# Dizzy-cell/HOUV

Measured on AMD Instinct MI355X. Metric: registration pairs/sec (2048-pt partial pairs), higher is better.
Workload: dtype f32; 1 GPU; HOUV solve_model, 2048x2048-pt pairs, batch 256/GPU, K=64 restarts x 200 Adam iterations + retry stages (BASELINE configs[1]); pairs_per_gpu=256, points=2048, kernel=64, iters=200, icp_refine=False, parallelism=dp1 (pair shards, one RCCL all-gather of [steps*P,12] per rank)

## Files before the change

### houv_amd/csrc/capi.hip

```cpp
#include <stdarg.h>
#include <string.h>

#include "../../include/houv_hip.h"
#include "houv_common.h"

namespace houv {

static thread_local char g_err[512] = "";

void set_error(const char* fmt, ...) {
  va_list ap;
  va_start(ap, fmt);
  vsnprintf(g_err, sizeof(g_err), fmt, ap);
  va_end(ap);
  fprintf(stderr, "[houv_hip] %s\n", g_err);
}

DebugKnobs g_debug;

namespace {

__global__ void pose_kernel(const float* __restrict__ params, int n, int angle_base, int trans_mode,
                            float* __restrict__ R, float* __restrict__ T) {
  const int i = blockIdx.x * blockDim.x + threadIdx.x;
  if (i >= n) return;
  float p[8];
#pragma unroll
  for (int k = 0; k < 8; ++k) p[k] = params[i * 8 + k];
  Pose f;
  pose_forward(p, angle_base, trans_mode, f);
#pragma unroll
  for (int k = 0; k < 9; ++k) R[i * 9 + k] = f.R[k];
#pragma unroll
  for (int k = 0; k < 3; ++k) T[i * 3 + k] = f.T[k];
}

__global__ void move_kernel(const float* __restrict__ src, const float* __restrict__ R, const float* __restrict__ T,
                            size_t total, int N, float* __restrict__ moved) {
  for (size_t e = (size_t)blockIdx.x * blockDim.x + threadIdx.x; e < total; e += (size_t)gridDim.x * blockDim.x) {
    const size_t b = e / N;
    const float* r = R + b * 9;
    const float x = src[e * 3 + 0], y = src[e * 3 + 1], z = src[e * 3 + 2];
    moved[e * 3 + 0] = __builtin_fmaf(z, r[2], __builtin_fmaf(y, r[1], x * r[0])) + T[b * 3 + 0];
    moved[e * 3 + 1] = __builtin_fmaf(z, r[5], __builtin_fmaf(y, r[4], x * r[3])) + T[b * 3 + 1];
    moved[e * 3 + 2] = __builtin_fmaf(z, r[8], __builtin_fmaf(y, r[7], x * r[6])) + T[b * 3 + 2];
  }
}

}
}

extern "C" int houv_abi_version(void) { return HOUV_ABI_VERSION; }

extern "C" const char* houv_last_error(void) { return houv::g_err; }

extern "C" int houv_debug_set(const char* name, long long value) {
  using namespace houv;
  const struct { const char* name; std::atomic<int>* knob; long long lo, hi, step; } ints[] = {
      {"solve_predict", &g_debug.pred_mode, 0, 2, 1}, {"knn_split", &g_debug.knn_split, 0, 1, 1},
      {"attn_split", &g_debug.attn_split, 0, 1, 1},   {"gemm_split", &g_debug.gemm_split, 0, 6, 3}};
  if (name && !strcmp(name, "solve_stats")) {
    g_debug.stats = (unsigned long long)value;
    return 1;
  }
  if (name && !strcmp(name, "solve_walk_hist")) {
    g_debug.walk_hist = (unsigned long long)value;
    return 1;
  }
  if (name && !strcmp(name, "solve_cull_stats")) {
    g_debug.cull_stats = (unsigned long long)value;
    return 1;
  }
  for (const auto& k : ints)
    if (name && !strcmp(name, k.name) && value >= k.lo && value <= k.hi && value % k.step == 0) {
      *k.knob = (int)value;
      return 1;
    }
  set_error("houv_debug_set: unknown switch or value out of range: %s = %lld", name ? name : "(null)", value);
  return 0;
}

#ifndef HOUV_BUILD_ID
#define HOUV_BUILD_ID "unknown"
#endif
extern "C" const char* houv_build_id(void) { return HOUV_BUILD_ID; }

extern "C" int houv_pose_forward(const float* params, int n, int angle_base, int trans_mode, const float* src, int N,
                                 float* R, float* T, float* moved, void* stream) {
  using namespace houv;
  if (n < 0 || !params || !R || !T || angle_base < 0 || angle_base > 3 || trans_mode < 0 || trans_mode > 1) {
    set_error("houv_pose_forward: bad argument");
    return 0;
  }
  if (n == 0) return 1;
  hipStream_t s = (hipStream_t)stream;
  pose_kernel<<<(n + 255) / 256, 256, 0, s>>>(params, n, angle_base, trans_mode, R, T);
  if (src && moved && N > 0) {
    const size_t total = (size_t)n * N;
    size_t blocks = (total + 255) / 256;
    if (blocks > 16384) blocks = 16384;
    move_kernel<<<(unsigned)blocks, 256, 0, s>>>(src, R, T, total, N, moved);
  }
  return check_launch("houv_pose_forward") ? 1 : 0;
}
```

### houv_amd/csrc/houv_common.h

```cpp
#pragma once
#include <hip/hip_runtime.h>
#include <stdint.h>
#include <stdio.h>

#include <atomic>

#include "houv_math.h"

namespace houv {

constexpr int kWave = 64;
constexpr int kSub = 32;
constexpr int kTrk = 16;

void set_error(const char* fmt, ...);
struct SolveCommon;
__attribute__((visibility("hidden"))) int solve_check_args(const char* who, const SolveCommon& a, int use_views);
__attribute__((visibility("hidden"))) bool scatter_index_launch(const int* keys, int B, int N, int M, int* offsets, int* order,
                                                                hipStream_t stream);
inline bool check_launch(const char* what) {
  hipError_t e = hipGetLastError();
  if (e != hipSuccess) {
    set_error("%s: %s", what, hipGetErrorString(e));
    return false;
  }
  return true;
}

struct DebugKnobs {
  std::atomic<int> pred_mode{0};
  std::atomic<unsigned long long> stats{0ull};
  std::atomic<unsigned long long> walk_hist{0ull};
  std::atomic<unsigned long long> cull_stats{0ull};
  std::atomic<int> knn_split{1};
  std::atomic<int> attn_split{1};
  std::atomic<int> gemm_split{6};
};
extern DebugKnobs g_debug;

template <int MET>
__device__ __forceinline__ float metric_sqdist(float dx, float dy, float dz) {
  if constexpr (MET == 0) return __builtin_fmaf(dz, dz, __builtin_fmaf(dy, dy, dx * dx));
  else if constexpr (MET == 1) return __builtin_fmaf(dz, dz, dy * dy);
  else if constexpr (MET == 2) return __builtin_fmaf(dz, dz, dx * dx);
  else return __builtin_fmaf(dy, dy, dx * dx);
}

__device__ __forceinline__ float min3f(float a, float b, float c) {
  return __builtin_fminf(__builtin_fminf(a, b), c);
}

__device__ __forceinline__ float wave_sum(float v) {
#pragma unroll
  for (int o = 32; o > 0; o >>= 1) v += __shfl_xor(v, o, kWave);
  return v;
}

__device__ __forceinline__ int wave_sum_i(int v) {
#pragma unroll
  for (int o = 32; o > 0; o >>= 1) v += __shfl_xor(v, o, kWave);
  return v;
}

template <int CTRL, int ROW_MASK = 0xf, int BANK_MASK = 0xf>
__device__ __forceinline__ float dpp_f(float v) {
  return __int_as_float(__builtin_amdgcn_update_dpp(0, __float_as_int(v), CTRL, ROW_MASK, BANK_MASK, true));
}
template <int CTRL, int ROW_MASK = 0xf, int BANK_MASK = 0xf>
__device__ __forceinline__ int dpp_i(int v) {
  return __builtin_amdgcn_update_dpp(0, v, CTRL, ROW_MASK, BANK_MASK, true);
}

__device__ __forceinline__ float wave_sum_to_lane63(float v) {
  v += dpp_f<0x111>(v);
  v += dpp_f<0x112>(v);
  v += dpp_f<0x114>(v);
  v += dpp_f<0x118>(v);
  v += dpp_f<0x142, 0xa>(v);
  v += dpp_f<0x143, 0xc>(v);
  return v;
}

__device__ __forceinline__ int wave_max_to_lane63(int v) {
  v = max(v, dpp_i<0x111>(v));
  v = max(v, dpp_i<0x112>(v));
  v = max(v, dpp_i<0x114>(v));
  v = max(v, dpp_i<0x118>(v));
  v = max(v, dpp_i<0x142, 0xa>(v));
  v = max(v, dpp_i<0x143, 0xc>(v));
  return v;
}

template <int CTRL, int ROW_MASK = 0xf>
__device__ __forceinline__ float fmax_dpp(float v) {
  return __builtin_fmaxf(v, __int_as_float(__builtin_amdgcn_update_dpp(__float_as_int(v), __float_as_int(v), CTRL, ROW_MASK, 0xf, false)));
}
__device__ __forceinline__ float wave_fmax_to_lane63(float v) {
  v = fmax_dpp<0x111>(v);
  v = fmax_dpp<0x112>(v);
  v = fmax_dpp<0x114>(v);
  v = fmax_dpp<0x118>(v);
  v = fmax_dpp<0x142, 0xa>(v);
  v = fmax_dpp<0x143, 0xc>(v);
  return v;
}

__device__ __forceinline__ int wave_incl_scan_dpp(int x) {
  int v = x + dpp_i<0x111>(x);
  v += dpp_i<0x112>(x);
  v += dpp_i<0x113>(x);
  v += dpp_i<0x114, 0xf, 0xe>(v);
  v += dpp_i<0x118, 0xf, 0xc>(v);
  v += dpp_i<0x142, 0xa>(v);
  v += dpp_i<0x143, 0xc>(v);
  return v;
}

__device__ __forceinline__ int wave_incl_scan_i(int v) {
  const int lane = threadIdx.x & 63;
#pragma unroll
  for (int o = 1; o < 64; o <<= 1) {
    int n = __shfl_up(v, o, kWave);
    if (lane >= o) v += n;
  }
  return v;
}

}
```

### houv_amd/csrc/houv_solve.h

```cpp
#pragma once
#include <stddef.h>

#include "houv_sweep.h"

namespace houv {

struct SolveCommon {
  const float* src;
  const float* tgt;
  int P, N, M, K;
  double* state;
  int steps_done, n_iters, angle_base, trans_mode, f64_params, k_full, k_view;
  double lr, beta1, beta2, eps;
  float loss_scale;
  float* out_score;
  float* out_loss;
  float* out_R;
  float* out_T;
  float* out_grad;
  float* out_cd;
};

constexpr int kRedStride = 4 * kAccN;
constexpr int kHistBins = 256;
constexpr int kHistSets = 3;
constexpr int kPoseFloats = 28;
static_assert(sizeof(Pose) <= kPoseFloats * 4 && offsetof(Pose, T) == 36, "pose[0..11] in LDS must be R | T");

__device__ __forceinline__ void store_pose(float* dst, const Pose& f) {
  const float* src = reinterpret_cast<const float*>(&f);
#pragma unroll
  for (int i = 0; i < (int)(sizeof(Pose) / 4); ++i) dst[i] = src[i];
}
__device__ __forceinline__ void load_pose(Pose& f, const float* src) {
  float* dst = reinterpret_cast<float*>(&f);
#pragma unroll
  for (int i = 0; i < (int)(sizeof(Pose) / 4); ++i) dst[i] = src[i];
}
__device__ __forceinline__ void load_rt(const float* pose, float (&R)[9], float (&T)[3]) {
#pragma unroll
  for (int i = 0; i < 9; ++i) R[i] = pose[i];
#pragma unroll
  for (int i = 0; i < 3; ++i) T[i] = pose[9 + i];
}

__device__ __forceinline__ void move_point(const float (&R)[9], const float (&T)[3], float sx, float sy, float sz, float& mx,
                                           float& my, float& mz) {
  mx = __builtin_fmaf(sz, R[2], __builtin_fmaf(sy, R[1], sx * R[0])) + T[0];
  my = __builtin_fmaf(sz, R[5], __builtin_fmaf(sy, R[4], sx * R[3])) + T[1];
  mz = __builtin_fmaf(sz, R[8], __builtin_fmaf(sy, R[7], sx * R[6])) + T[2];
}

__device__ __forceinline__ void store_outputs(float* out_score, float* out_loss, float* out_R, float* out_T, float* out_grad,
                                              float* out_cd, int inst, const Pose& f, const TailLoss& r) {
  if (out_score) out_score[inst] = r.score;
  if (out_loss) out_loss[inst] = r.loss;
  if (out_R)
    for (int k = 0; k < 9; ++k) out_R[(size_t)inst * 9 + k] = f.R[k];
  if (out_T)
    for (int k = 0; k < 3; ++k) out_T[(size_t)inst * 3 + k] = f.T[k];
  if (out_grad)
    for (int k = 0; k < 8; ++k) out_grad[(size_t)inst * 8 + k] = r.g[k];
  if (out_cd)
    for (int m = 0; m < 4; ++m)
      for (int d = 0; d < 2; ++d) out_cd[(size_t)inst * 8 + m * 2 + d] = r.cd[m][d];
}

struct RadixState {
  unsigned prefix, mask;
  int remaining, neq;
};

template <int BLOCK>
__device__ __forceinline__ unsigned* radix_rotate(unsigned* hist, int& hrot, int tid) {
  unsigned* h = hist + hrot * kHistBins;
  hrot = (hrot == kHistSets - 1) ? 0 : hrot + 1;
  for (int i = tid; i < kHistBins; i += BLOCK) hist[hrot * kHistBins + i] = 0u;
  return h;
}

__device__ __forceinline__ void radix_count(unsigned* h, unsigned key, int pass, int lane, const RadixState& s) {
  if (pass == 0) {
    const unsigned digit = key >> 24;
    unsigned long long todo = __ballot(1);
    while (todo) {
      const int leader = __ffsll((long long)todo) - 1;
      const unsigned d = (unsigned)__builtin_amdgcn_readlane((int)digit, leader);
      const unsigned long long m = __ballot(digit == d);
      if (lane == leader) atomicAdd(&h[d], (unsigned)__popcll(m));
      todo &= ~m;
    }
  } else if ((key & s.mask) == s.prefix) {
    atomicAdd(&h[(key >> (24 - 8 * pass)) & 255u], 1u);
  }
}

__device__ __forceinline__ void radix_pick(const unsigned* h, int pass, int lane, RadixState& s) {
  const int shift = 24 - 8 * pass;
  const uint4 hv = *reinterpret_cast<const uint4*>(h + 4 * lane);
  const int hh[4] = {(int)hv.x, (int)hv.y, (int)hv.z, (int)hv.w};
  const int tot = hh[0] + hh[1] + hh[2] + hh[3];
  int c = wave_incl_scan_dpp(tot) - tot;
  int fbin = 0, fc = 0, fn = 0;
  bool found = false;
#pragma unroll
  for (int b = 0; b < 4; ++b) {
    const bool hit = c < s.remaining && s.remaining <= c + hh[b];
    fbin = hit ? 4 * lane + b : fbin;
    fc = hit ? c : fc;
    fn = hit ? hh[b] : fn;
    found = found || hit;
    c += hh[b];
  }
  const int src_lane = __ffsll((long long)__ballot(found)) - 1;
  const int bin = __builtin_amdgcn_readlane(fbin, src_lane);
  s.prefix |= (unsigned)bin << shift;
  s.mask |= 255u << shift;
  s.remaining -= __builtin_amdgcn_readlane(fc, src_lane);
  s.neq = __builtin_amdgcn_readlane(fn, src_lane);
}

}
```

### houv_amd/csrc/solve.hip

```cpp
#include <stddef.h>
#include <stdlib.h>

#include "../../include/houv_hip.h"
#include "houv_common.h"
#include "houv_solve.h"

namespace houv {
namespace {

struct SolveArgs : SolveCommon {
  short* nn_ws;
  int ws_valid;
  int ws_stride;
  int pred_mode;
  unsigned long long* stats;
  unsigned long long* walk_hist;
  unsigned long long* cull_stats;
};

constexpr int kRescanBatch = 4;
constexpr int kRefresh = 4;
constexpr int kTermMaxAge = 0;

struct Smem {
  float4* tgt;
  float4* mov;
  double* state;
  double* adam;
  float* pose;
  float* acc;
  float* red;
  unsigned* hist;
  int* ctl;
  float4* tbox;
  float4* mbox;
  SortedStage st;
  float* anchor;
};
constexpr int kAnchorFloats = kTermAnchorFloats + 4;
constexpr int kTermAges = 8;
constexpr int kStalePose = 4;


__host__ __device__ inline int pad_unit(int prune) { return prune == 3 ? 2 * kSub : kSub; }

__host__ __device__ inline size_t smem_bytes(int N, int M, int block, int prune, int q) {
  const int pu = pad_unit(prune);
  int npad = (N + pu - 1) / pu * pu, mpad = (M + pu - 1) / pu * pu;
  if (prune) npad = mpad = (npad > mpad ? npad : mpad);
  const int nw = block / 64;
  const size_t nq = (size_t)block * q;
  return (size_t)(npad + mpad) * 16 + 28 * 8 + kPoseFloats * 4 + 8 * kAccStride * 4 + (size_t)2 * nw * kRedStride * 4 +
         kHistSets * kHistBins * 4 + (8 + nw) * 4 + 64 + (prune ? 2 * 128 * 16 + nq * 2 + 132 * 4 + kAnchorFloats * 4 : 0);
}

__device__ inline Smem carve(unsigned char* base, int N, int M, int block, int nq, int pu) {
  int npad = (N + pu - 1) / pu * pu, mpad = (M + pu - 1) / pu * pu;
  if (nq) npad = mpad = (npad > mpad ? npad : mpad);
  const int nw = block / 64;
  Smem s;
  s.tgt = reinterpret_cast<float4*>(base);
  s.mov = s.tgt + mpad;
  s.state = reinterpret_cast<double*>(s.mov + npad);
  s.adam = s.state + 24;
  s.pose = reinterpret_cast<float*>(s.adam + 4);
  s.acc = s.pose + kPoseFloats;
  s.red = s.acc + 8 * kAccStride;
  s.hist = reinterpret_cast<unsigned*>(s.red + 2 * nw * kRedStride);
  s.ctl = reinterpret_cast<int*>(s.hist + kHistSets * kHistBins);
  const size_t box_off = ((size_t)(reinterpret_cast<unsigned char*>(s.ctl + 8 + nw) - base) + 15) & ~(size_t)15;
  s.tbox = reinterpret_cast<float4*>(base + box_off);
  s.mbox = s.tbox + 128;
  s.st.hist = reinterpret_cast<int*>(s.mbox + 128);
  s.st.order = reinterpret_cast<unsigned short*>(s.st.hist + 132);
  s.anchor = reinterpret_cast<float*>(s.st.order + nq);
  return s;
}

template <typename T>
__device__ __forceinline__ T fresh(T v) {
  asm volatile("" : "+s"(v));
  return v;
}
__device__ __forceinline__ const float* fresh_lds(const float* p) {
  typedef const float __attribute__((address_space(3))) * lds_f;
  return (const float*)(lds_f)(size_t)fresh((unsigned)(size_t)(lds_f)p);
}

template <int BLOCK, int Q>
__device__ __forceinline__ void select_smallest(const unsigned (&key)[Q], int ksel, unsigned* hist, int* ctl,
                                                bool (&sel)[Q], int& hrot) {
  constexpr int NW = BLOCK / 64;
  const int tid = tid_x(), lane = tid & 63, wave = tid >> 6;
  RadixState rs{0u, 0u, ksel, 0};
#pragma unroll
  for (int pass = 0; pass < 4; ++pass) {
    unsigned* h = radix_rotate<BLOCK>(hist, hrot, tid);
#pragma unroll
    for (int k = 0; k < Q; ++k) radix_count(h, key[k], pass, lane, rs);
    __syncthreads();
    radix_pick(h, pass, lane, rs);
  }
  const unsigned prefix = rs.prefix;
  const int remaining = rs.remaining, neq = rs.neq;
  if (neq == remaining) {
#pragma unroll
    for (int k = 0; k < Q; ++k) sel[k] = key[k] <= prefix;
  } else {
    int e = 0;
#pragma unroll
    for (int k = 0; k < Q; ++k) e += (key[k] == prefix) ? 1 : 0;
    const int incl = wave_incl_scan_dpp(e);
    __syncthreads();
    if (lane == 63) ctl[8 + wave] = incl;
    __syncthreads();
    int rank = incl - e;
    for (int w = 0; w < NW; ++w) rank += (w < wave) ? ctl[8 + w] : 0;
#pragma unroll
    for (int k = 0; k < Q; ++k) {
      const bool eq = key[k] == prefix;
      sel[k] = key[k] < prefix || (eq && rank < remaining);
      rank += eq ? 1 : 0;
    }
  }
}

constexpr int kGradN = 12;

__device__ __forceinline__ void park(float v, float* dst) {
  v = wave_sum_to_lane63(v);
  if ((tid_x() & 63) == 63) *dst = v;
}

template <int BLOCK, int Q, int NMET>
__device__ __forceinline__ void select_all(const Smem& sm, const float (&best)[Q][NMET], int count, int k_full, int k_view,
                                           unsigned need, int& hrot, unsigned (&bits)[NMET]) {
  bool valid[Q], sel[Q];
  unsigned key[Q];
#pragma unroll
  for (int m = 0; m < NMET; ++m) {
    const int ksel = (m == 0) ? k_full : k_view;
#pragma unroll
    for (int k = 0; k < Q; ++k) {
      valid[k] = pt_index<BLOCK>(k) < count;
      key[k] = valid[k] ? __float_as_uint(best[k][m]) : 0xFFFFFFFFu;
      sel[k] = valid[k];
    }
    if (ksel < count && ((need >> m) & 1u)) select_smallest<BLOCK, Q>(key, ksel, sm.hist, sm.ctl, sel, hrot);
    unsigned b = 0u;
#pragma unroll
    for (int k = 0; k < Q; ++k) b |= sel[k] ? (1u << k) : 0u;
    bits[m] = b;
  }
}

template <int Q>
__device__ __forceinline__ float lane_sqrt_sum(const float (&bd)[Q], unsigned selbits) {
  float s = 0.f;
#pragma unroll
  for (int k = 0; k < Q; ++k)
    if ((selbits >> k) & 1u) s += (bd[k] < INFINITY) ? sqrtf(bd[k]) : NAN;
  return s;
}

template <int BLOCK, int Q, int MET, int DIR, bool WS>
__device__ __forceinline__ void lane_grad_sums(const Smem& sm, const float4* __restrict__ refs, const float (&qx)[Q],
                                               const float (&qy)[Q], const float (&qz)[Q], const float (&bd)[Q],
                                               const int (&bt)[Q], unsigned selbits, int count, const float (&px)[Q],
                                               const float (&py)[Q], const float (&pz)[Q], float (&g)[kGradN], buf_t ws,
                                               int ws_off) {
  const int rot = tid_x() & (kSub - 1);
#pragma unroll
  for (int i = 0; i < kGradN; ++i) g[i] = 0.f;
  float R[9], T[3];
  if constexpr (DIR == 0) load_rt(sm.pose, R, T);
#pragma unroll
  for (int k = 0; k < Q; ++k) {
    int jn;
    const float4 nn = recover_nn<MET, kRescanBatch, true>(refs + bt[k] * kTrk, qx[k], qy[k], qz[k], bd[k], rot, jn);
    if (WS && pt_index<BLOCK>(k) < count)
      __builtin_amdgcn_raw_buffer_store_b16((unsigned short)(bt[k] * kTrk + jn), ws, tid_x() * kNnRec,
                                            ws_off + pt_base<BLOCK>(k) * kNnRec + MET * 2, 0);
    if ((selbits >> k) & 1u) {
      const float s = (bd[k] < INFINITY) ? sqrtf(bd[k]) : NAN;
      const float inv = 1.0f / s;
      float dx, dy, dz, sx, sy, sz;
      if constexpr (DIR == 1) {
        dx = qx[k] - nn.x; dy = qy[k] - nn.y; dz = qz[k] - nn.z;
        sx = px[k]; sy = py[k]; sz = pz[k];
      } else {
        dx = nn.x - qx[k]; dy = nn.y - qy[k]; dz = nn.z - qz[k];
        const float ux = nn.x - T[0], uy = nn.y - T[1], uz = nn.z - T[2];
        sx = R[0] * ux + R[3] * uy + R[6] * uz;
        sy = R[1] * ux + R[4] * uy + R[7] * uz;
        sz = R[2] * ux + R[5] * uy + R[8] * uz;
      }
      if constexpr (MET == 1) dx = 0.f;
      if constexpr (MET == 2) dy = 0.f;
      if constexpr (MET == 3) dz = 0.f;
      const float cx = dx * inv, cy = dy * inv, cz = dz * inv;
      g[0] += cx; g[1] += cy; g[2] += cz;
      g[3] += cx * sx; g[4] += cx * sy; g[5] += cx * sz;
      g[6] += cy * sx; g[7] += cy * sy; g[8] += cy * sz;
      g[9] += cz * sx; g[10] += cz * sy; g[11] += cz * sz;
    }
  }
}

template <int BLOCK, int Q, int NMET>
__device__ __forceinline__ void park_sqrt_sums(const float (&best)[Q][NMET], const unsigned (&selbits)[NMET], unsigned need,
                                               float* red_wave) {
  float bd[Q];
#pragma unroll
  for (int m = 0; m < NMET; ++m) {
    if (!((need >> m) & 1u)) continue;
#pragma unroll
    for (int k = 0; k < Q; ++k) bd[k] = best[k][m];
    park(lane_sqrt_sum<Q>(bd, selbits[m]), red_wave + m * kAccN);
  }
}

template <int BLOCK, int Q, int NMET, int DIR, bool WS>
__device__ __forceinline__ void park_grad_sums(const Smem& sm, const float4* __restrict__ refs, const float (&qx)[Q],
                                               const float (&qy)[Q], const float (&qz)[Q], const float (&best)[Q][NMET],
                                               const int (&btile)[Q][NMET], const unsigned (&selbits)[NMET], unsigned mask,
                                               int count, const float (&px)[Q], const float (&py)[Q], const float (&pz)[Q],
                                               float* red_wave, buf_t ws, int ws_off) {
  float bd[Q], g[kGradN];
  int bt[Q];
#define HOUV_GRAD(MET)                                                                                              \
  if ((mask >> MET) & 1u) {                                                                                         \
    _Pragma("unroll") for (int k = 0; k < Q; ++k) {                                                                 \
      bd[k] = best[k][MET];                                                                                         \
      bt[k] = btile[k][MET];                                                                                        \
    }                                                                                                               \
    lane_grad_sums<BLOCK, Q, MET, DIR, WS>(sm, refs, qx, qy, qz, bd, bt, selbits[MET], count, px, py, pz, g,        \
                                           ws, ws_off);                                                             \
    _Pragma("unroll") for (int i = 0; i < kGradN; ++i) park(g[i], red_wave + MET * kAccN + 1 + i);                  \
  }
  HOUV_GRAD(0)
  if constexpr (NMET == 4) {
    HOUV_GRAD(1)
    HOUV_GRAD(2)
    HOUV_GRAD(3)
  }
#undef HOUV_GRAD
}

template <int BLOCK, int NMET>
__device__ __forceinline__ void final_sums(const Smem& sm, int dir, bool want_s, unsigned grad_mask, unsigned need) {
  constexpr int NW = BLOCK / 64;
  const int tid = tid_x();
  if (tid < NMET * kAccN) {
    const int m = tid / kAccN, i = tid % kAccN;
    if ((i == 0) ? want_s : (((grad_mask >> m) & 1u) != 0u)) {
      const float* r = sm.red + (size_t)dir * NW * kRedStride + tid;
      float a = 0.f;
#pragma unroll
      for (int w = 0; w < NW; ++w) a += r[w * kRedStride];
      if (i == 0 && !((need >> m) & 1u)) a = INFINITY;
      sm.acc[(m * 2 + dir) * kAccStride + i] = a;
    }
  }
}

template <int NMET>
__device__ __forceinline__ unsigned picked_direction(const Smem& sm, int k_full, int k_view) {
  unsigned pick = 0u;
#pragma unroll
  for (int m = 0; m < NMET; ++m) {
    const float kk = (float)((m == 0) ? k_full : k_view);
    const float cd0 = sm.acc[(m * 2 + 0) * kAccStride] / kk, cd1 = sm.acc[(m * 2 + 1) * kAccStride] / kk;
    pick |= (cd0 <= cd1) ? 0u : (1u << m);
  }
  return pick;
}

template <int BLOCK>
__device__ __forceinline__ void load_src_point(buf_t src, int k, int N, float& x, float& y, float& z) {
  x = y = z = 0.f;
  if (pt_index<BLOCK>(k) < N) {
    const auto v = __builtin_amdgcn_raw_buffer_load_b96(src, tid_x() * 12, pt_base<BLOCK>(k) * 12, 0);
    x = __uint_as_float(v[0]); y = __uint_as_float(v[1]); z = __uint_as_float(v[2]);
  }
}

template <int BLOCK, int Q, int MET>
__device__ __forceinline__ void repair_direction_a(const Smem& sm, buf_t src, int N, int mpad, int k_sel,
                                                   int& hrot, float* red_wave) {
  float sx[Q], sy[Q], sz[Q], mx[Q], my[Q], mz[Q];
  float R[9], T[3];
  load_rt(sm.pose, R, T);
#pragma unroll
  for (int k = 0; k < Q; ++k) {
    load_src_point<BLOCK>(src, k, N, sx[k], sy[k], sz[k]);
    move_point(R, T, sx[k], sy[k], sz[k], mx[k], my[k], mz[k]);
  }
  float bd[Q];
  int bt[Q];
  sweep_one<Q, MET>(sm.tgt, mpad / kTrk, mx, my, mz, bd, bt);
  bool sel[Q];
  unsigned key[Q], bits = 0u;
#pragma unroll
  for (int k = 0; k < Q; ++k) {
    sel[k] = pt_index<BLOCK>(k) < N;
    key[k] = sel[k] ? __float_as_uint(bd[k]) : 0xFFFFFFFFu;
  }
  if (k_sel < N) select_smallest<BLOCK, Q>(key, k_sel, sm.hist, sm.ctl, sel, hrot);
#pragma unroll
  for (int k = 0; k < Q; ++k) bits |= sel[k] ? (1u << k) : 0u;
  float g[kGradN];
  lane_grad_sums<BLOCK, Q, MET, 1, false>(sm, sm.tgt, mx, my, mz, bd, bt, bits, N, sx, sy, sz, g, src, 0);
#pragma unroll
  for (int i = 0; i < kGradN; ++i) park(g[i], red_wave + MET * kAccN + 1 + i);
}

template <int BLOCK, int Q, int NMET, int PRUNE>
__global__ __launch_bounds__(BLOCK, (Q == 1 ? 8 : 4)) void solve_kernel(SolveArgs a) {
  static_assert(PRUNE == 0 || PRUNE == 2 || PRUNE == 3, "brute force, or the balanced walk over sub-tiles / super-tiles");
  constexpr int TS = (PRUNE == 3) ? 1 : 0;
  constexpr int kPad = kSub << TS;
  extern __shared__ __attribute__((aligned(512))) unsigned char smem_raw[];
  const int N = a.N, M = a.M;
  const Smem sm = carve(smem_raw, N, M, BLOCK, PRUNE ? BLOCK * Q : 0, kPad);
  const int tid = tid_x();
  const int ninst = a.P * a.K;
  int inst = blockIdx.x;
  if ((ninst & 7) == 0) inst = (blockIdx.x & 7) * (ninst >> 3) + (blockIdx.x >> 3);
  const int pair = inst / a.K;
  const buf_t src = make_buf(a.src + (size_t)pair * N * 3, N * 12);
  const float* __restrict__ tgt = a.tgt + (size_t)pair * M * 3;
  const int npad = (N + kPad - 1) / kPad * kPad, mpad = (M + kPad - 1) / kPad * kPad;
  const float4 pad4 = make_float4(INFINITY, INFINITY, INFINITY, 0.f);

  for (int j = tid; j < mpad; j += BLOCK) sm.tgt[j] = (j < M) ? make_float4(tgt[j * 3], tgt[j * 3 + 1], tgt[j * 3 + 2], 0.f) : pad4;
  for (int j = N + tid; j < npad; j += BLOCK) sm.mov[j] = pad4;
  if (tid < 24) sm.state[tid] = a.state[(size_t)inst * 24 + tid];
  for (int j = tid; j < kHistBins; j += BLOCK) sm.hist[j] = 0u;
  if constexpr (PRUNE) {
    if (tid < 132) sm.st.hist[tid] = 0;
  }
  int hrot = 0;
  __syncthreads();
  buf_t ws = src;
  const int ws_b = 0, ws_a = a.ws_stride * kNnRec;
  float4* ws_res = nullptr;
  if constexpr (PRUNE) {
    ws = make_buf(a.nn_ws + (size_t)inst * 16 * a.ws_stride, 32 * a.ws_stride);
    ws_res = reinterpret_cast<float4*>(a.nn_ws + ((size_t)inst * 16 + 8) * a.ws_stride);
    float tx0[Q], ty0[Q], tz0[Q];
#pragma unroll
    for (int k = 0; k < Q; ++k) {
      const int i = pt_index<BLOCK>(k);
      const float4 v = (i < M) ? sm.tgt[i] : make_float4(0.f, 0.f, 0.f, 0.f);
      tx0[k] = v.x; ty0[k] = v.y; tz0[k] = v.z;
    }
    tile_boxes<BLOCK, Q, TS>(tx0, ty0, tz0, M, mpad / kPad, sm.tbox);
  }
  constexpr int kAdamTid = BLOCK >= 128 ? 64 : 0;
  if (tid == 0) {
    float p[8];
#pragma unroll
    for (int k = 0; k < 8; ++k) p[k] = (float)sm.state[k];
    Pose f;
    pose_forward(p, a.angle_base, a.trans_mode, f);
    store_pose(sm.pose, f);
  }
  if (tid == kAdamTid) {
    const int step = a.steps_done + 1;
    const AdamScalars asc = adam_scalars(step, a.lr, a.beta1, a.beta2);
    sm.adam[(step & 1) * 2 + 0] = asc.step_size;
    sm.adam[(step & 1) * 2 + 1] = asc.bc2_sqrt;
  }
  if constexpr (PRUNE) {
    float r2 = 0.f;
#pragma unroll
    for (int k = 0; k < Q; ++k) {
      float x, y, z;
      load_src_point<BLOCK>(src, k, N, x, y, z);
      const float v = __builtin_fmaf(z, z, __builtin_fmaf(y, y, x * x));
      r2 = (v <= r2) ? r2 : ((v < INFINITY) ? v : INFINITY);
    }
#pragma unroll
    for (int o = 1; o < 64; o <<= 1) r2 = fmaxf(r2, __shfl_xor(r2, o, 64));
    if ((tid & 63) == 0) sm.red[tid >> 6] = r2;
    if (tid == 0) {
      sm.ctl[0] = (int)(((1u << NMET) - 1u) * 0x11u);
      reinterpret_cast<unsigned*>(sm.anchor)[kTermAges] = 0u;
    }
  }
  __syncthreads();
  if constexpr (PRUNE) {
    if (tid == 0) {
      float r2 = 0.f;
      for (int w = 0; w < BLOCK / 64; ++w) r2 = fmaxf(r2, sm.red[w]);
      sm.anchor[kTermAnchorFloats] = sqrtf(r2) * 1.000001f;
    }
  }

  unsigned long long clk0 = 0ull, rt0 = 0ull;
  if (a.stats) {
    clk0 = __builtin_amdgcn_s_memtime();
    rt0 = __builtin_amdgcn_s_memrealtime();
  }
  constexpr int NW = BLOCK / 64;
  constexpr unsigned kAllMet = (1u << NMET) - 1u;
  unsigned pred_a = kAllMet;
  auto red_row = [&](int dir) { return sm.red + ((size_t)dir * NW + (tid_x() >> 6)) * kRedStride; };
#pragma unroll 1
  for (int it = 0; it < a.n_iters; ++it) {
    if (a.pred_mode == 1) pred_a = 0u;
    const bool allgrad = a.pred_mode == 2 || ((PRUNE != 0) && (((a.steps_done + it) % kRefresh) == 0 || (a.ws_valid == 0 && it == 0)));
    unsigned need_a = kAllMet, need_b = kAllMet;
    if constexpr (PRUNE != 0) {
      const unsigned w = (unsigned)__builtin_amdgcn_readfirstlane(*reinterpret_cast<const int*>(fresh_lds(reinterpret_cast<const float*>(sm.ctl))));
      need_b = w & kAllMet;
      need_a = (w >> 4) & kAllMet;
    }
    const unsigned grad_a = (allgrad ? kAllMet : (pred_a | ~need_b)) & need_a;
    {
      float sx[Q], sy[Q], sz[Q], mx[Q], my[Q], mz[Q];
      float R[9], T[3];
      load_rt(fresh_lds(sm.pose), R, T);
#pragma unroll
      for (int k = 0; k < Q; ++k) {
        const int i = pt_index<BLOCK>(k);
        const bool ok = i < N;
        load_src_point<BLOCK>(src, k, N, sx[k], sy[k], sz[k]);
        move_point(R, T, sx[k], sy[k], sz[k], mx[k], my[k], mz[k]);
        if (ok) sm.mov[i] = make_float4(mx[k], my[k], mz[k], 0.f);
      }
      __syncthreads();
      bool pruned_now = false;
      float best[Q][NMET];
      int btile[Q][NMET];
      if constexpr (PRUNE) {
        tile_boxes<BLOCK, Q, TS>(mx, my, mz, N, npad / kPad, sm.mbox);
        pruned_now = (a.ws_valid != 0) || (it > 0);
      }
      if (need_a != 0u) {
        if (pruned_now) {
          if constexpr (PRUNE != 0)
            pruned_sweep_sorted<BLOCK, Q, NMET, TS>(sm.tgt, sm.tbox, mpad / kPad, sm.mbox, sm.mov, sm.tgt, sm.mov, mx, my, mz, ws, ws_a, N,
                                                need_a, sm.st, ws_res, best, btile, a.stats, fresh(a.walk_hist), fresh(a.cull_stats));
        } else {
          sweep<Q, NMET>(sm.tgt, mpad / kTrk, mx, my, mz, best, btile);
          if (a.stats && (tid & 63) == 0) atomicAdd(&a.stats[3], 1ull);
        }
        unsigned sel[NMET];
        select_all<BLOCK, Q, NMET>(sm, best, N, a.k_full, a.k_view, need_a, hrot, sel);
        park_sqrt_sums<BLOCK, Q, NMET>(best, sel, need_a, red_row(1));
        park_grad_sums<BLOCK, Q, NMET, 1, PRUNE != 0>(sm, sm.tgt, mx, my, mz, best, btile, sel, grad_a, N, sx, sy, sz, red_row(1), ws,
                                                     ws_a);
      }
      __syncthreads();
      final_sums<BLOCK, NMET>(sm, 1, true, grad_a, need_a);
    }
    unsigned pick_a;
    {
      float tx[Q], ty[Q], tz[Q];
#pragma unroll
      for (int k = 0; k < Q; ++k) {
        const int i = pt_index<BLOCK>(k);
        const float4 v = (i < M) ? sm.tgt[i] : make_float4(0.f, 0.f, 0.f, 0.f);
        tx[k] = v.x; ty[k] = v.y; tz[k] = v.z;
      }
      const bool pruned_now = (PRUNE != 0) && ((a.ws_valid != 0) || (it > 0));
      auto pick_winners = [&]() {
        __syncthreads();
        final_sums<BLOCK, NMET>(sm, 0, true, 0u, need_b);
        __syncthreads();
        pick_a = picked_direction<NMET>(sm, fresh(a.k_full), fresh(a.k_view));
        return (allgrad ? kAllMet : (~pick_a & kAllMet)) & need_b;
      };
      unsigned grad_b = 0u;
      if (need_b != 0u) {
        float best[Q][NMET];
        int btile[Q][NMET];
        if (pruned_now) {
          if constexpr (PRUNE != 0)
            pruned_sweep_sorted<BLOCK, Q, NMET, TS>(sm.mov, sm.mbox, npad / kPad, sm.tbox, sm.tgt, sm.tgt, sm.mov, tx, ty, tz, ws, ws_b, M,
                                                need_b, sm.st, ws_res, best, btile, a.stats, fresh(a.walk_hist), fresh(a.cull_stats));
        } else {
          sweep<Q, NMET>(sm.mov, npad / kTrk, tx, ty, tz, best, btile);
          if (a.stats && (tid & 63) == 0) atomicAdd(&a.stats[3], 1ull);
        }
        unsigned sel[NMET];
        select_all<BLOCK, Q, NMET>(sm, best, M, a.k_full, a.k_view, need_b, hrot, sel);
        park_sqrt_sums<BLOCK, Q, NMET>(best, sel, need_b, red_row(0));
        grad_b = pick_winners();
        park_grad_sums<BLOCK, Q, NMET, 0, PRUNE != 0>(sm, sm.mov, tx, ty, tz, best, btile, sel, grad_b, M, tx, ty, tz, red_row(0), ws,
                                                     ws_b);
      } else {
        pick_winners();
      }
      const unsigned miss = pick_a & ~grad_a & kAllMet;
      if (miss) {
        if (miss & 1u) repair_direction_a<BLOCK, Q, 0>(sm, src, N, mpad, a.k_full, hrot, red_row(1));
        if constexpr (NMET == 4) {
          if (miss & 2u) repair_direction_a<BLOCK, Q, 1>(sm, src, N, mpad, a.k_view, hrot, red_row(1));
          if (miss & 4u) repair_direction_a<BLOCK, Q, 2>(sm, src, N, mpad, a.k_view, hrot, red_row(1));
          if (miss & 8u) repair_direction_a<BLOCK, Q, 3>(sm, src, N, mpad, a.k_view, hrot, red_row(1));
        }
      }
      __syncthreads();
      final_sums<BLOCK, NMET>(sm, 0, false, grad_b, kAllMet);
      if (miss) final_sums<BLOCK, NMET>(sm, 1, false, miss, kAllMet);
    }
    pred_a = pick_a;
    static_assert(NMET * kAccN <= 64, "final_sums runs on the scalar tail's wave");
    __builtin_amdgcn_wave_barrier();

    if (kAdamTid != 0 && tid == kAdamTid && it + 1 < a.n_iters) {
      const int step = a.steps_done + it + 2;
      const AdamScalars asc = adam_scalars(step, fresh(a.lr), fresh(a.beta1), fresh(a.beta2));
      sm.adam[(step & 1) * 2 + 0] = asc.step_size;
      sm.adam[(step & 1) * 2 + 1] = asc.bc2_sqrt;
    }
    if (tid == 0) {
      const int k_full = fresh(a.k_full), k_view = fresh(a.k_view);
      const float loss_scale = fresh(a.loss_scale);
      const double lr = fresh(a.lr), beta1 = fresh(a.beta1), beta2 = fresh(a.beta2), eps = fresh(a.eps);
      const int angle_base = fresh(a.angle_base), trans_mode = fresh(a.trans_mode);
      Pose f;
      load_pose(f, sm.pose);
      TailLoss r;
      solve_tail_loss<NMET>(sm.acc, kAccStride, f, k_full, k_view, loss_scale, trans_mode, r);
      if (it == a.n_iters - 1)
        store_outputs(a.out_score, a.out_loss, a.out_R, a.out_T, a.out_grad, a.out_cd, inst, f, r);
      if constexpr (PRUNE != 0) {
#pragma unroll
        for (int m = 0; m < NMET; ++m) {
          if ((need_b >> m) & 1u) sm.anchor[2 * m] = r.cd[m][0];
          if ((need_a >> m) & 1u) sm.anchor[2 * m + 1] = r.cd[m][1];
        }
      }
      const int step = a.steps_done + it + 1;
      const AdamScalars asc{sm.adam[(step & 1) * 2 + 0], sm.adam[(step & 1) * 2 + 1]};
      solve_tail_step(r.g, sm.state, a.f64_params, asc, beta1, beta2, eps, angle_base, trans_mode, f);
      if constexpr (PRUNE != 0) {
        unsigned next = kAllMet | (kAllMet << 4), ages = 0u;
        const bool all_next = fresh(a.pred_mode) == 2 || it + 2 >= a.n_iters;
        if (!all_next) {
          const unsigned have = need_b | (need_a << 4);
          float* stale = reinterpret_cast<float*>(sm.tbox) + 3;
          next = term_anchor_masks<NMET>(sm.anchor, sm.pose, stale, kStalePose, ~have & 0xffu, f.R, f.T,
                                         sm.anchor[kTermAnchorFloats]);
          const unsigned old_ages = reinterpret_cast<const unsigned*>(sm.anchor)[kTermAges];
#pragma unroll
          for (int m = 0; m < NMET; ++m) {
            unsigned age = (old_ages >> (8 * m)) & 0xffu;
            age = (((next >> m) & (next >> (4 + m)) & 1u) != 0u) ? 0u : age + 1u;
            if (kTermMaxAge > 0 && age > (unsigned)kTermMaxAge) {
              next |= 0x11u << m;
              age = 0u;
            }
            if (age > 0xffu) age = 0xffu;
            ages |= age << (8 * m);
            if (((have & ~next) >> m) & 0x11u) {
#pragma unroll
              for (int i = 0; i < 12; ++i) stale[(m * 12 + i) * kStalePose] = sm.pose[i];
            }
          }
        }
        reinterpret_cast<unsigned*>(sm.anchor)[kTermAges] = ages;
        sm.ctl[0] = (int)next;
        if (a.stats) {
          atomicAdd(&a.stats[6], (unsigned long long)(__popc(need_a) + __popc(need_b)));
          atomicAdd(&a.stats[7], (unsigned long long)(2 * NMET));
        }
      }
      store_pose(sm.pose, f);
      if (kAdamTid == 0 && it + 1 < a.n_iters) {
        const AdamScalars nxt = adam_scalars(step + 1, lr, beta1, beta2);
        sm.adam[((step + 1) & 1) * 2 + 0] = nxt.step_size;
        sm.adam[((step + 1) & 1) * 2 + 1] = nxt.bc2_sqrt;
      }
    }
    __syncthreads();
  }
  if (tid_x() < 24) a.state[(size_t)inst * 24 + tid_x()] = sm.state[tid_x()];
  if (a.stats) {
    const unsigned long long dc = __builtin_amdgcn_s_memtime() - clk0, dr = __builtin_amdgcn_s_memrealtime() - rt0;
    if (tid == 0) {
      atomicAdd(&a.stats[4], dc);
      atomicAdd(&a.stats[5], dr);
    }
  }
}

template <int BLOCK, int Q, int PRUNE>
int launch(const SolveArgs& a, int use_views, hipStream_t s) {
  const size_t bytes = smem_bytes(a.N, a.M, BLOCK, PRUNE, Q);
  const int grid = a.P * a.K;
  hipError_t e;
  if (use_views) {
    e = hipFuncSetAttribute((const void*)solve_kernel<BLOCK, Q, 4, PRUNE>, hipFuncAttributeMaxDynamicSharedMemorySize, (int)bytes);
    if (e != hipSuccess) { set_error("houv_solve_iterate: cannot reserve %zu B of LDS: %s", bytes, hipGetErrorString(e)); return 0; }
    solve_kernel<BLOCK, Q, 4, PRUNE><<<grid, BLOCK, bytes, s>>>(a);
  } else {
    e = hipFuncSetAttribute((const void*)solve_kernel<BLOCK, Q, 1, PRUNE>, hipFuncAttributeMaxDynamicSharedMemorySize, (int)bytes);
    if (e != hipSuccess) { set_error("houv_solve_iterate: cannot reserve %zu B of LDS: %s", bytes, hipGetErrorString(e)); return 0; }
    solve_kernel<BLOCK, Q, 1, PRUNE><<<grid, BLOCK, bytes, s>>>(a);
  }
  return check_launch("houv_solve_iterate") ? 1 : 0;
}

}
}

extern "C" int houv_solve_variant(int N, int M, int pruned, int* block, int* points_per_lane, int* prune_mode) {
  using namespace houv;
  const int mx = N > M ? N : M;
  if (N <= 0 || M <= 0) {
    set_error("houv_solve_variant: bad cloud sizes N=%d M=%d", N, M);
    return 0;
  }
  if (mx > 4096) {
    set_error("houv_solve_iterate: clouds larger than 4096 points do not fit in 160 KiB of LDS (N=%d M=%d)", N, M);
    return 0;
  }
  int b, q;
  if (mx <= 64) { b = 64; q = 1; }
  else if (mx <= 128) { b = 128; q = 1; }
  else if (mx <= 256) { b = 256; q = 1; }
  else if (mx <= 512) { b = 256; q = 2; }
  else if (mx <= 768) { b = 256; q = 3; }
  else if (mx <= 1024) { b = 256; q = 4; }
  else if (mx <= 1536) { b = 512; q = 3; }
  else if (mx <= 2048) { b = 512; q = 4; }
  else if (mx <= 3072) { b = 1024; q = 3; }
  else { b = 1024; q = 4; }
  if (block) *block = b;
  if (points_per_lane) *points_per_lane = q;
  constexpr int kPrunedMinPoints = 257;
  if (prune_mode) *prune_mode = (!pruned || mx < kPrunedMinPoints) ? 0 : (mx > 2048) ? 3 : 2;
  return 1;
}

extern "C" int houv_solve_walk_variant(int need) {
  if (need < 0 || need > 15) {
    houv::set_error("houv_solve_walk_variant: the term mask of a direction is 0..15, got %d", need);
    return -1;
  }
  return (int)houv::walk_variant((unsigned)need);
}

extern "C" long long houv_solve_lds_bytes(int N, int M, int pruned) {
  using namespace houv;
  int block = 0, q = 0, mode = 0;
  if (!houv_solve_variant(N, M, pruned, &block, &q, &mode)) return -1;
  return (long long)smem_bytes(N, M, block, mode, q);
}

int houv::solve_check_args(const char* who, const SolveCommon& a, int use_views) {
  const int P = a.P, N = a.N, M = a.M;
  if (P < 0 || N <= 0 || M <= 0 || a.K <= 0 || a.n_iters <= 0 || a.steps_done < 0 || a.angle_base < 0 || a.angle_base > 3 ||
      a.trans_mode < 0 || a.trans_mode > 1) {
    set_error("%s: bad argument P=%d N=%d M=%d K=%d n_iters=%d steps_done=%d base=%d trans_mode=%d", who, P, N, M, a.K,
              a.n_iters, a.steps_done, a.angle_base, a.trans_mode);
    return 0;
  }
  if (P == 0) return 1;
  if (!a.src || !a.tgt || !a.state) {
    set_error("%s: null pointer", who);
    return 0;
  }
  const int kv = use_views ? a.k_view : 1;
  if (a.k_full < 1 || a.k_full > N || a.k_full > M || kv < 1 || kv > N || kv > M) {
    set_error("%s: top-k size out of range (k_full=%d k_view=%d N=%d M=%d)", who, a.k_full, a.k_view, N, M);
    return 0;
  }
  if ((long long)P * a.K > 0x7fffffffLL) {
    set_error("%s: too many hypotheses", who);
    return 0;
  }
  return 2;
}

static int solve_dispatch(const houv::SolveCommon& c, int use_views, short* nn_ws, int ws_valid, int ws_stride, bool prune,
                          void* stream, const char* who) {
  using namespace houv;
  const int ok = solve_check_args(who, c, use_views);
  if (ok < 2) return ok;
  const int N = c.N, M = c.M;
  SolveArgs a{c, nn_ws, ws_valid, ws_stride, g_debug.pred_mode.load(),
              reinterpret_cast<unsigned long long*>(g_debug.stats.load()),
              reinterpret_cast<unsigned long long*>(g_debug.walk_hist.load()),
              reinterpret_cast<unsigned long long*>(g_debug.cull_stats.load())};
  hipStream_t s = (hipStream_t)stream;
  const int mx = N > M ? N : M;
  int block = 0, q = 0, mode = 0;
  if (!houv_solve_variant(N, M, prune ? 1 : 0, &block, &q, &mode)) return 0;
  if (prune && (!nn_ws || ws_stride < mx || (ws_stride & 7))) {
    set_error("%s: pruned mode needs a workspace of 16 x ws_stride int16 per hypothesis, ws_stride >= max(N,M) and a multiple of 8", who);
    return 0;
  }
  if (prune && ((uintptr_t)nn_ws & 15)) {
    set_error("%s: the pruned-mode workspace must be 16-byte aligned", who);
    return 0;
  }
  if (prune && ws_valid < 0) {
    a.ws_valid = 0;
    mode = 0;
  }
  if (mode == 0) a.nn_ws = nullptr;
#define HOUV_GO(B_, Q_)                                                          \
  if (block == B_ && q == Q_) {                                                  \
    if (mode == 2) return launch<B_, Q_, ((B_ >= 256 && Q_ >= 2) ? 2 : 0)>(a, use_views, s);    \
    return launch<B_, Q_, 0>(a, use_views, s);                                   \
  }
  if (mx <= 2048) {
    HOUV_GO(64, 1) HOUV_GO(128, 1) HOUV_GO(256, 1) HOUV_GO(256, 2) HOUV_GO(256, 3) HOUV_GO(256, 4)
    HOUV_GO(512, 3) HOUV_GO(512, 4)
  } else {
    if (block == 1024 && q == 3) return mode == 3 ? launch<1024, 3, 3>(a, use_views, s) : launch<1024, 3, 0>(a, use_views, s);
    if (block == 1024 && q == 4) return mode == 3 ? launch<1024, 4, 3>(a, use_views, s) : launch<1024, 4, 0>(a, use_views, s);
  }
#undef HOUV_GO
  set_error("%s: no kernel variant <%d,%d>", who, block, q);
  return 0;
}

extern "C" int houv_solve_iterate(const float* src, const float* tgt, int P, int N, int M, int K, double* state,
                                  int steps_done, int n_iters, int angle_base, int trans_mode, int use_views,
                                  int f64_params, int k_full, int k_view, double lr, double beta1, double beta2,
                                  double eps, float loss_scale, float* out_score, float* out_loss, float* out_R,
                                  float* out_T, float* out_grad, float* out_cd, void* stream) {
  const houv::SolveCommon a{src, tgt, P, N, M, K, state, steps_done, n_iters, angle_base, trans_mode, f64_params, k_full, k_view,
                            lr, beta1, beta2, eps, loss_scale, out_score, out_loss, out_R, out_T, out_grad, out_cd};
  return solve_dispatch(a, use_views, nullptr, 0, 0, false, stream, "houv_solve_iterate");
}

extern "C" int houv_solve_iterate_pruned(const float* src, const float* tgt, int P, int N, int M, int K, double* state,
                                         int steps_done, int n_iters, int angle_base, int trans_mode, int use_views,
                                         int f64_params, int k_full, int k_view, double lr, double beta1, double beta2,
                                         double eps, float loss_scale, float* out_score, float* out_loss, float* out_R,
                                         float* out_T, float* out_grad, float* out_cd, int16_t* nn_ws, int ws_valid,
                                         int ws_stride, void* stream) {
  const houv::SolveCommon a{src, tgt, P, N, M, K, state, steps_done, n_iters, angle_base, trans_mode, f64_params, k_full, k_view,
                            lr, beta1, beta2, eps, loss_scale, out_score, out_loss, out_R, out_T, out_grad, out_cd};
  return solve_dispatch(a, use_views, (short*)nn_ws, ws_valid, ws_stride, true, stream, "houv_solve_iterate_pruned");
}
```

Baseline: 215.1 pairs/s.

## Seed radix top-k select with the previous iteration's top byte and prune repair sweeps

The radix selection for the full metric now remembers the top byte of the previous threshold per direction. It tries one combined pass that counts keys below that guess and builds a 16-bit histogram of the guessed bucket, skipping the first two radix passes when the guess holds. The direction-A repair path also uses the pruned sorted sweep when pruning is active, where before it always ran a brute-force rescan. A debug counter for repair events is added. The risks are extra LDS control slots, an atomic and a barrier per guessed select, and falling back to the full passes when the guess misses.

```diff
diff --git a/houv_amd/csrc/capi.hip b/houv_amd/csrc/capi.hip
--- a/houv_amd/csrc/capi.hip
+++ b/houv_amd/csrc/capi.hip
@@ -71,6 +71,10 @@
     g_debug.cull_stats = (unsigned long long)value;
     return 1;
   }
+  if (name && !strcmp(name, "solve_repair_stats")) {
+    g_debug.repair_stats = (unsigned long long)value;
+    return 1;
+  }
   for (const auto& k : ints)
     if (name && !strcmp(name, k.name) && value >= k.lo && value <= k.hi && value % k.step == 0) {
       *k.knob = (int)value;
diff --git a/houv_amd/csrc/houv_common.h b/houv_amd/csrc/houv_common.h
--- a/houv_amd/csrc/houv_common.h
+++ b/houv_amd/csrc/houv_common.h
@@ -32,6 +32,7 @@
   std::atomic<unsigned long long> stats{0ull};
   std::atomic<unsigned long long> walk_hist{0ull};
   std::atomic<unsigned long long> cull_stats{0ull};
+  std::atomic<unsigned long long> repair_stats{0ull};
   std::atomic<int> knn_split{1};
   std::atomic<int> attn_split{1};
   std::atomic<int> gemm_split{6};
diff --git a/houv_amd/csrc/houv_solve.h b/houv_amd/csrc/houv_solve.h
--- a/houv_amd/csrc/houv_solve.h
+++ b/houv_amd/csrc/houv_solve.h
@@ -95,8 +95,8 @@
   }
 }
 
-__device__ __forceinline__ void radix_pick(const unsigned* h, int pass, int lane, RadixState& s) {
-  const int shift = 24 - 8 * pass;
+__device__ __forceinline__ unsigned long long radix_find(const unsigned* h, int lane, int remaining, int& bin, int& before,
+                                                         int& count) {
   const uint4 hv = *reinterpret_cast<const uint4*>(h + 4 * lane);
   const int hh[4] = {(int)hv.x, (int)hv.y, (int)hv.z, (int)hv.w};
   const int tot = hh[0] + hh[1] + hh[2] + hh[3];
@@ -105,19 +105,45 @@
   bool found = false;
 #pragma unroll
   for (int b = 0; b < 4; ++b) {
-    const bool hit = c < s.remaining && s.remaining <= c + hh[b];
+    const bool hit = c < remaining && remaining <= c + hh[b];
     fbin = hit ? 4 * lane + b : fbin;
     fc = hit ? c : fc;
     fn = hit ? hh[b] : fn;
     found = found || hit;
     c += hh[b];
   }
-  const int src_lane = __ffsll((long long)__ballot(found)) - 1;
-  const int bin = __builtin_amdgcn_readlane(fbin, src_lane);
+  const unsigned long long where = __ballot(found);
+  const int src_lane = (__ffsll((long long)where) - 1) & 63;
+  bin = __builtin_amdgcn_readlane(fbin, src_lane);
+  before = __builtin_amdgcn_readlane(fc, src_lane);
+  count = __builtin_amdgcn_readlane(fn, src_lane);
+  return where;
+}
+
+__device__ __forceinline__ void radix_pick(const unsigned* h, int pass, int lane, RadixState& s) {
+  const int shift = 24 - 8 * pass;
+  int bin, before, count;
+  radix_find(h, lane, s.remaining, bin, before, count);
   s.prefix |= (unsigned)bin << shift;
   s.mask |= 255u << shift;
-  s.remaining -= __builtin_amdgcn_readlane(fc, src_lane);
-  s.neq = __builtin_amdgcn_readlane(fn, src_lane);
+  s.remaining -= before;
+  s.neq = count;
+}
+
+__device__ __forceinline__ void radix_count_guess(unsigned* h, unsigned key, unsigned g, int& below) {
+  const unsigned top = key >> 24;
+  below += __popcll(__ballot(top < g));
+  if (top == g) atomicAdd(&h[(key >> 16) & 255u], 1u);
+}
+
+__device__ __forceinline__ bool radix_pick_guess(const unsigned* h, int lane, unsigned g, int ksel, int below, RadixState& s) {
+  int bin, before, count;
+  if (radix_find(h, lane, ksel - below, bin, before, count) == 0ull) return false;
+  s.prefix = (g << 24) | ((unsigned)bin << 16);
+  s.mask = 0xFFFF0000u;
+  s.remaining = ksel - below - before;
+  s.neq = count;
+  return true;
 }
 
 }
diff --git a/houv_amd/csrc/solve.hip b/houv_amd/csrc/solve.hip
--- a/houv_amd/csrc/solve.hip
+++ b/houv_amd/csrc/solve.hip
@@ -16,6 +16,7 @@
   unsigned long long* stats;
   unsigned long long* walk_hist;
   unsigned long long* cull_stats;
+  unsigned long long* repair_stats;
 };
 
 constexpr int kRescanBatch = 4;
@@ -37,6 +38,7 @@
   SortedStage st;
   float* anchor;
 };
+constexpr int kCtlBelow = 1, kCtlGuess = 2;
 constexpr int kAnchorFloats = kTermAnchorFloats + 4;
 constexpr int kTermAges = 8;
 constexpr int kStalePose = 4;
@@ -87,20 +89,37 @@
   return (const float*)(lds_f)(size_t)fresh((unsigned)(size_t)(lds_f)p);
 }
 
-template <int BLOCK, int Q>
+template <int BLOCK, int Q, int GSLOT = -1>
 __device__ __forceinline__ void select_smallest(const unsigned (&key)[Q], int ksel, unsigned* hist, int* ctl,
                                                 bool (&sel)[Q], int& hrot) {
   constexpr int NW = BLOCK / 64;
   const int tid = tid_x(), lane = tid & 63, wave = tid >> 6;
   RadixState rs{0u, 0u, ksel, 0};
+  bool tried = false, hit = false;
+  if constexpr (GSLOT >= 0) {
+    const int g = __builtin_amdgcn_readfirstlane(ctl[GSLOT]);
+    if (g >= 0) {
+      tried = true;
+      unsigned* h = radix_rotate<BLOCK>(hist, hrot, tid);
+      int below = 0;
+#pragma unroll
+      for (int k = 0; k < Q; ++k) radix_count_guess(h, key[k], (unsigned)g, below);
+      if (lane == 0) atomicAdd(&ctl[kCtlBelow], below);
+      __syncthreads();
+      hit = radix_pick_guess(h, lane, (unsigned)g, ksel, __builtin_amdgcn_readfirstlane(ctl[kCtlBelow]), rs);
+    }
+  }
 #pragma unroll
   for (int pass = 0; pass < 4; ++pass) {
+    if (pass < 2 && hit) continue;
     unsigned* h = radix_rotate<BLOCK>(hist, hrot, tid);
+    if (GSLOT >= 0 && pass == 3 && tried && tid == 0) ctl[kCtlBelow] = 0;
 #pragma unroll
     for (int k = 0; k < Q; ++k) radix_count(h, key[k], pass, lane, rs);
     __syncthreads();
     radix_pick(h, pass, lane, rs);
   }
+  if (GSLOT >= 0 && tid == 0) ctl[GSLOT] = (int)(rs.prefix >> 24);
   const unsigned prefix = rs.prefix;
   const int remaining = rs.remaining, neq = rs.neq;
   if (neq == remaining) {
@@ -132,7 +151,7 @@
   if ((tid_x() & 63) == 63) *dst = v;
 }
 
-template <int BLOCK, int Q, int NMET>
+template <int BLOCK, int Q, int NMET, int DIR>
 __device__ __forceinline__ void select_all(const Smem& sm, const float (&best)[Q][NMET], int count, int k_full, int k_view,
                                            unsigned need, int& hrot, unsigned (&bits)[NMET]) {
   bool valid[Q], sel[Q];
@@ -146,7 +165,10 @@
       key[k] = valid[k] ? __float_as_uint(best[k][m]) : 0xFFFFFFFFu;
       sel[k] = valid[k];
     }
-    if (ksel < count && ((need >> m) & 1u)) select_smallest<BLOCK, Q>(key, ksel, sm.hist, sm.ctl, sel, hrot);
+    if (ksel < count && ((need >> m) & 1u)) {
+      if (m == 0) select_smallest<BLOCK, Q, kCtlGuess + DIR>(key, ksel, sm.hist, sm.ctl, sel, hrot);
+      else select_smallest<BLOCK, Q>(key, ksel, sm.hist, sm.ctl, sel, hrot);
+    }
     unsigned b = 0u;
 #pragma unroll
     for (int k = 0; k < Q; ++k) b |= sel[k] ? (1u << k) : 0u;
@@ -306,13 +328,57 @@
     sel[k] = pt_index<BLOCK>(k) < N;
     key[k] = sel[k] ? __float_as_uint(bd[k]) : 0xFFFFFFFFu;
   }
-  if (k_sel < N) select_smallest<BLOCK, Q>(key, k_sel, sm.hist, sm.ctl, sel, hrot);
+  if (k_sel < N) select_smallest<BLOCK, Q, (MET == 0 ? kCtlGuess + 1 : -1)>(key, k_sel, sm.hist, sm.ctl, sel, hrot);
 #pragma unroll
   for (int k = 0; k < Q; ++k) bits |= sel[k] ? (1u << k) : 0u;
   float g[kGradN];
   lane_grad_sums<BLOCK, Q, MET, 1, false>(sm, sm.tgt, mx, my, mz, bd, bt, bits, N, sx, sy, sz, g, src, 0);
 #pragma unroll
   for (int i = 0; i < kGradN; ++i) park(g[i], red_wave + MET * kAccN + 1 + i);
+}
+
+template <int BLOCK, int Q, int NMET, int TS>
+__device__ __forceinline__ void repair_direction_a_pruned(const Smem& sm, buf_t src, int N, int ntile, unsigned miss, int k_full,
+                                                          int k_view, int& hrot, float* red_wave, buf_t ws, int ws_a,
+                                                          float4* ws_res) {
+  float sx[Q], sy[Q], sz[Q], mx[Q], my[Q], mz[Q];
+  float R[9], T[3];
+  load_rt(sm.pose, R, T);
+#pragma unroll
+  for (int k = 0; k < Q; ++k) {
+    load_src_point<BLOCK>(src, k, N, sx[k], sy[k], sz[k]);
+    move_point(R, T, sx[k], sy[k], sz[k], mx[k], my[k], mz[k]);
+  }
+  float best[Q][NMET];
+  int btile[Q][NMET];
+  pruned_sweep_sorted<BLOCK, Q, NMET, TS>(sm.tgt, sm.tbox, ntile, sm.mbox, sm.mov, sm.tgt, sm.mov, mx, my, mz, ws, ws_a, N, miss, sm.st,
+                                          ws_res, best, btile, nullptr, nullptr, nullptr);
+  float bd[Q], g[kGradN];
+  int bt[Q];
+  bool sel[Q];
+  unsigned key[Q];
+#define HOUV_REPAIR(MET)                                                                                            \
+  if ((miss >> MET) & 1u) {                                                                                         \
+    const int k_sel = (MET == 0) ? k_full : k_view;                                                                 \
+    unsigned bits = 0u;                                                                                             \
+    _Pragma("unroll") for (int k = 0; k < Q; ++k) {                                                                 \
+      bd[k] = best[k][MET];                                                                                         \
+      bt[k] = btile[k][MET];                                                                                        \
+      sel[k] = pt_index<BLOCK>(k) < N;                                                                              \
+      key[k] = sel[k] ? __float_as_uint(bd[k]) : 0xFFFFFFFFu;                                                       \
+    }                                                                                                               \
+    if (k_sel < N) select_smallest<BLOCK, Q, (MET == 0 ? kCtlGuess + 1 : -1)>(key, k_sel, sm.hist, sm.ctl, sel, hrot); \
+    _Pragma("unroll") for (int k = 0; k < Q; ++k) bits |= sel[k] ? (1u << k) : 0u;                                   \
+    lane_grad_sums<BLOCK, Q, MET, 1, false>(sm, sm.tgt, mx, my, mz, bd, bt, bits, N, sx, sy, sz, g, src, 0);        \
+    _Pragma("unroll") for (int i = 0; i < kGradN; ++i) park(g[i], red_wave + MET * kAccN + 1 + i);                  \
+  }
+  HOUV_REPAIR(0)
+  if constexpr (NMET == 4) {
+    HOUV_REPAIR(1)
+    HOUV_REPAIR(2)
+    HOUV_REPAIR(3)
+  }
+#undef HOUV_REPAIR
 }
 
 template <int BLOCK, int Q, int NMET, int PRUNE>
@@ -337,6 +403,7 @@
   for (int j = N + tid; j < npad; j += BLOCK) sm.mov[j] = pad4;
   if (tid < 24) sm.state[tid] = a.state[(size_t)inst * 24 + tid];
   for (int j = tid; j < kHistBins; j += BLOCK) sm.hist[j] = 0u;
+  if (tid >= kCtlBelow && tid < kCtlGuess + 2) sm.ctl[tid] = (tid == kCtlBelow) ? 0 : -1;
   if constexpr (PRUNE) {
     if (tid < 132) sm.st.hist[tid] = 0;
   }
@@ -448,7 +515,7 @@
           if (a.stats && (tid & 63) == 0) atomicAdd(&a.stats[3], 1ull);
         }
         unsigned sel[NMET];
-        select_all<BLOCK, Q, NMET>(sm, best, N, a.k_full, a.k_view, need_a, hrot, sel);
+        select_all<BLOCK, Q, NMET, 1>(sm, best, N, a.k_full, a.k_view, need_a, hrot, sel);
         park_sqrt_sums<BLOCK, Q, NMET>(best, sel, need_a, red_row(1));
         park_grad_sums<BLOCK, Q, NMET, 1, PRUNE != 0>(sm, sm.tgt, mx, my, mz, best, btile, sel, grad_a, N, sx, sy, sz, red_row(1), ws,
                                                      ws_a);
@@ -486,7 +553,7 @@
           if (a.stats && (tid & 63) == 0) atomicAdd(&a.stats[3], 1ull);
         }
         unsigned sel[NMET];
-        select_all<BLOCK, Q, NMET>(sm, best, M, a.k_full, a.k_view, need_b, hrot, sel);
+        select_all<BLOCK, Q, NMET, 0>(sm, best, M, a.k_full, a.k_view, need_b, hrot, sel);
         park_sqrt_sums<BLOCK, Q, NMET>(best, sel, need_b, red_row(0));
         grad_b = pick_winners();
         park_grad_sums<BLOCK, Q, NMET, 0, PRUNE != 0>(sm, sm.mov, tx, ty, tz, best, btile, sel, grad_b, M, tx, ty, tz, red_row(0), ws,
@@ -496,11 +563,21 @@
       }
       const unsigned miss = pick_a & ~grad_a & kAllMet;
       if (miss) {
-        if (miss & 1u) repair_direction_a<BLOCK, Q, 0>(sm, src, N, mpad, a.k_full, hrot, red_row(1));
-        if constexpr (NMET == 4) {
-          if (miss & 2u) repair_direction_a<BLOCK, Q, 1>(sm, src, N, mpad, a.k_view, hrot, red_row(1));
-          if (miss & 4u) repair_direction_a<BLOCK, Q, 2>(sm, src, N, mpad, a.k_view, hrot, red_row(1));
-          if (miss & 8u) repair_direction_a<BLOCK, Q, 3>(sm, src, N, mpad, a.k_view, hrot, red_row(1));
+        if (unsigned long long* rs = fresh(a.repair_stats); rs && tid == 0) {
+          atomicAdd(&rs[0], 1ull);
+          atomicAdd(&rs[1], (unsigned long long)__popc(miss));
+        }
+        if (pruned_now) {
+          if constexpr (PRUNE != 0)
+            repair_direction_a_pruned<BLOCK, Q, NMET, TS>(sm, src, N, mpad / kPad, miss, fresh(a.k_full), fresh(a.k_view), hrot,
+                                                          red_row(1), ws, ws_a, ws_res);
+        } else {
+          if (miss & 1u) repair_direction_a<BLOCK, Q, 0>(sm, src, N, mpad, a.k_full, hrot, red_row(1));
+          if constexpr (NMET == 4) {
+            if (miss & 2u) repair_direction_a<BLOCK, Q, 1>(sm, src, N, mpad, a.k_view, hrot, red_row(1));
+            if (miss & 4u) repair_direction_a<BLOCK, Q, 2>(sm, src, N, mpad, a.k_view, hrot, red_row(1));
+            if (miss & 8u) repair_direction_a<BLOCK, Q, 3>(sm, src, N, mpad, a.k_view, hrot, red_row(1));
+          }
         }
       }
       __syncthreads();
@@ -687,7 +764,8 @@
   SolveArgs a{c, nn_ws, ws_valid, ws_stride, g_debug.pred_mode.load(),
               reinterpret_cast<unsigned long long*>(g_debug.stats.load()),
               reinterpret_cast<unsigned long long*>(g_debug.walk_hist.load()),
-              reinterpret_cast<unsigned long long*>(g_debug.cull_stats.load())};
+              reinterpret_cast<unsigned long long*>(g_debug.cull_stats.load()),
+              reinterpret_cast<unsigned long long*>(g_debug.repair_stats.load())};
   hipStream_t s = (hipStream_t)stream;
   const int mx = N > M ? N : M;
   int block = 0, q = 0, mode = 0;
```

Result: no change. 216.6 pairs/s (median of 6 runs) (+0.7%).
